# CogSP/CoEvoNet

Hardware: NVIDIA B200
Metric: mpe_env_steps_per_sec (higher is better)
Workload: dtype f32

## Files before the change

coevonet_b200/csrc/rollout_lockstep.cu:

```cuda
#include <stdlib.h>

#include <cuda_fp16.h>

#include "rollout_common.cuh"
#include "tc_common.cuh"

namespace cev {

constexpr int LS_ST_FIELDS = 16;
constexpr int LS_OBS_PAD = 12;
constexpr int LS_L1S = 132;

struct LsBuffers {
    double* st;
    double* acc;
    float* min_gap;
    int32_t* goal;
    float* obs;
    int32_t* act;
    float* gap;
    __half* w2split;
    uint32_t* wmax;
    float* oscale;
    double* l1stats;
    float2* l1ms;
    double* ml1stats;
};

static size_t ls_align(size_t x) { return (x + 255) & ~(size_t)255; }

static size_t ls_carve(void* base, int64_t N, int K, int P, LsBuffers* b) {
    size_t off = 0;
    char* p = static_cast<char*>(base);
    auto take = [&](size_t bytes) {
        void* r = p ? p + off : nullptr;
        off += ls_align(bytes);
        return r;
    };
    LsBuffers t;
    t.w2split = static_cast<__half*>(take((size_t)2 * K * 2 * H2 * H1 * sizeof(__half)));
    t.wmax = static_cast<uint32_t*>(take((size_t)2 * K * sizeof(uint32_t)));
    t.oscale = static_cast<float*>(take((size_t)2 * K * 2 * sizeof(float)));
    t.st = static_cast<double*>(take((size_t)LS_ST_FIELDS * N * sizeof(double)));
    t.acc = static_cast<double*>(take((size_t)3 * N * sizeof(double)));
    t.min_gap = static_cast<float*>(take((size_t)N * sizeof(float)));
    t.goal = static_cast<int32_t*>(take((size_t)N * sizeof(int32_t)));
    t.obs = static_cast<float*>(take((size_t)3 * N * LS_OBS_PAD * sizeof(float)));
    t.act = static_cast<int32_t*>(take((size_t)3 * N * sizeof(int32_t)));
    t.gap = static_cast<float*>(take((size_t)3 * N * sizeof(float)));
    t.l1stats = static_cast<double*>(take((size_t)2 * K * LS_L1S * sizeof(double)));
    t.l1ms = static_cast<float2*>(take((size_t)2 * N * sizeof(float2)));
    t.ml1stats = static_cast<double*>(take((size_t)P * LS_L1S * sizeof(double)));
    if (b) *b = t;
    return off;
}

__device__ __forceinline__ void ls_store_state(const LsBuffers& b, int64_t N, int64_t ep, const EnvState& s) {
// ... 137 lines not shown
    p.b.acc[p.N + ep] = rg;
    p.b.acc[2 * p.N + ep] = sum_adv;
    p.b.min_gap[ep] = min_gap;
    ls_store_state(p.b, p.N, ep, s);
    if (!ls_store_obs(p.b, p.N, ep, s, p.K, p.E, p.opp_seat) && p.status) atomicOr(p.status, CEV_STATUS_NONFINITE);
}

struct LsPrepParams {
    const float* opp[2];
    int64_t opp_pitch[2];
    int seat[2];
    int K;
    __half* w2split;
    uint32_t* wmax;
    float* oscale;
    double* l1stats;
};

__device__ __forceinline__ int ls_scale_exp(float bound, int target) {
    if (!(bound > 0.f) || !isfinite(bound)) return 0;
    const int s = target - ilogbf(bound);
    return s < -40 ? -40 : (s > 40 ? 40 : s);
}

__global__ void __launch_bounds__(256) ls_wmax_kernel(const LsPrepParams p) {
    const int oi = blockIdx.y / p.K, k = blockIdx.y % p.K;
    const FcOffsets o = fc_offsets(seat_in_dim(p.seat[oi]));
    const float4* src = reinterpret_cast<const float4*>(p.opp[oi] + (int64_t)k * p.opp_pitch[oi] + o.fc2w);
    float m = 0.f;
    for (int f = blockIdx.x * blockDim.x + threadIdx.x; f < H2 * H1 / 4; f += gridDim.x * blockDim.x) {
// ... 62 lines not shown
        }
#pragma unroll
        for (int o = 16; o > 0; o >>= 1) s += __shfl_xor_sync(0xffffffffu, s, o);
        if (lane == 0) {
            out[11 + a * 11 + b] = s / H1;
            out[11 + b * 11 + a] = s / H1;
        }
    }
}

__global__ void __launch_bounds__(512) ls_l1stats_kernel(const LsPrepParams p) {
    const int oi = blockIdx.x / p.K, k = blockIdx.x % p.K;
    const int in = seat_in_dim(p.seat[oi]);
    const float* row = p.opp[oi] + (int64_t)k * p.opp_pitch[oi];
    ls_l1stats_row(row, in, p.l1stats + (size_t)blockIdx.x * LS_L1S);
    __shared__ float red[2][16];
    const int t = threadIdx.x;
    float g = fabsf(row[H1 * in + H1 + t]), be = fabsf(row[H1 * in + 2 * H1 + t]);
#pragma unroll
    for (int off = 16; off > 0; off >>= 1) {
        g = fmaxf(g, __shfl_xor_sync(0xffffffffu, g, off));
        be = fmaxf(be, __shfl_xor_sync(0xffffffffu, be, off));
    }
    if ((t & 31) == 0) {
        red[0][t >> 5] = g;
        red[1][t >> 5] = be;
    }
    __syncthreads();
    if (t == 0) {
        for (int w = 1; w < 16; ++w) {
            g = fmaxf(g, red[0][w]);
            be = fmaxf(be, red[1][w]);
        }
        const int sx = ls_scale_exp(22.63f * g + be, 13);
        const int sw = ls_scale_exp(__uint_as_float(p.wmax[blockIdx.x]), 14);
        p.oscale[blockIdx.x * 2 + 0] = ldexpf(1.0f, sx);
        p.oscale[blockIdx.x * 2 + 1] = ldexpf(1.0f, -(sx + sw));
    }
}

__global__ void __launch_bounds__(512) ls_member_l1stats_kernel(const float* __restrict__ members, int64_t pitch, int in,
                                                                double* __restrict__ out) {
    ls_l1stats_row(members + (int64_t)blockIdx.x * pitch, in, out + (size_t)blockIdx.x * LS_L1S);
}

#ifndef LS_GRID_OPP_DEFAULT
#define LS_GRID_OPP_DEFAULT 0
#endif
#ifndef LS_GRID_MEM_DEFAULT
#define LS_GRID_MEM_DEFAULT 0
#endif
constexpr int LS_BT = 16;
constexpr int LS_TAIL_FLOATS = 2056;
constexpr int LS_W1A_FLOATS = H1 * IN_GOOD + 3 * H1;

constexpr int OP_THREADS = 448;
constexpr int OP_PROD = 256;
constexpr int OP_BM = 128, OP_BN = 256, OP_BK = 64, OP_KT = H1 / OP_BK;
constexpr uint32_t OP_A_BYTES = OP_BM * OP_BK * 2;
constexpr uint32_t OP_B_BYTES = OP_BN * OP_BK * 2;
constexpr uint32_t OP_STAGE_BYTES = 2 * OP_A_BYTES + 2 * OP_B_BYTES;
constexpr int OP_STAGES = 2;
constexpr size_t OP_OFF_W1A = (size_t)OP_STAGES * OP_STAGE_BYTES;
constexpr size_t OP_OFF_TAIL = OP_OFF_W1A + (size_t)LS_W1A_FLOATS * 4;
constexpr size_t OP_OFF_BAR = OP_OFF_TAIL + (size_t)LS_TAIL_FLOATS * 4;
constexpr size_t OP_SMEM_MAX = 232448;
constexpr size_t OP_SLACK = OP_SMEM_MAX - (OP_OFF_BAR + 128);
constexpr size_t OP_SMEM = OP_SMEM_MAX;
constexpr uint32_t OP_IDESC = (1u << 4) | ((uint32_t)(OP_BN >> 3) << 17) | ((uint32_t)(OP_BM >> 4) << 24);

struct LsOppParams {
    const float* opp[2];
    int64_t opp_pitch[2];
    int seat[2];
    int K, E, n_tiles, n_jobs;
    int64_t PE;
    int64_t N;
    const float* obs;
    int32_t* act;
    float* gap;
    const float2* l1ms;
    const float* oscale;
    int32_t* status;
    float* logits;
};

template <int IN>
__device__ __forceinline__ void op_produce_chunk(const float* __restrict__ w1a, const float (&x)[4][IN_GOOD],
                                                 const float (&mean)[4], const float (&rstd)[4], float sx, int kt, int c,
                                                 int lane, unsigned char* __restrict__ a_hi,
                                                 unsigned char* __restrict__ a_lo) {
    const float* fc1b = w1a + H1 * IN;
    const float* ln1g = fc1b + H1;
    const float* ln1b = ln1g + H1;
    const int k0 = kt * OP_BK + c * 8;
    uint32_t hi[4][4], lo[4][4];
#pragma unroll
    for (int half = 0; half < 2; ++half) {
        const float4 bb = *reinterpret_cast<const float4*>(fc1b + k0 + 4 * half);
        const float4 gg = *reinterpret_cast<const float4*>(ln1g + k0 + 4 * half);
        const float4 ee = *reinterpret_cast<const float4*>(ln1b + k0 + 4 * half);
        const float bq[4] = {bb.x, bb.y, bb.z, bb.w}, gq[4] = {gg.x * sx, gg.y * sx, gg.z * sx, gg.w * sx},
                    eq[4] = {ee.x * sx, ee.y * sx, ee.z * sx, ee.w * sx};
        float hv[4][4];
#pragma unroll
        for (int qq = 0; qq < 4; ++qq) {
            float w[IN];
            const float2* wr = reinterpret_cast<const float2*>(w1a + (k0 + 4 * half + qq) * IN);
#pragma unroll
            for (int i2 = 0; i2 < IN / 2; ++i2) {
                const float2 v = wr[i2];
                w[2 * i2] = v.x;
                w[2 * i2 + 1] = v.y;
            }
#pragma unroll
            for (int j = 0; j < 4; ++j) {
                float pre = 0.f;
#pragma unroll
                for (int i = 0; i < IN; ++i) pre = fmaf(w[i], x[j][i], pre);
                pre += bq[qq];
                hv[j][qq] = fmaxf(fmaf((pre - mean[j]) * rstd[j], gq[qq], eq[qq]), 0.f);
            }
        }
#pragma unroll
        for (int j = 0; j < 4; ++j)
#pragma unroll
            for (int pr = 0; pr < 2; ++pr) {
                const __half2 h2 = __floats2half2_rn(hv[j][2 * pr], hv[j][2 * pr + 1]);
                const float2 hf = __half22float2(h2);
                const __half2 l2 = __floats2half2_rn(hv[j][2 * pr] - hf.x, hv[j][2 * pr + 1] - hf.y);
                hi[j][2 * half + pr] = *reinterpret_cast<const uint32_t*>(&h2);
                lo[j][2 * half + pr] = *reinterpret_cast<const uint32_t*>(&l2);
            }
    }
#pragma unroll
    for (int j = 0; j < 4; ++j) {
        const int r = lane + 32 * j;
        const int off = r * 128 + ((c ^ (r & 7)) << 4);
        *reinterpret_cast<uint4*>(a_hi + off) = make_uint4(hi[j][0], hi[j][1], hi[j][2], hi[j][3]);
        *reinterpret_cast<uint4*>(a_lo + off) = make_uint4(lo[j][0], lo[j][1], lo[j][2], lo[j][3]);
    }
}

struct Geo {
    static constexpr uint32_t B_BYTES = OP_B_BYTES;
    static constexpr uint32_t STAGE_BYTES = OP_STAGE_BYTES;
    static constexpr int STAGES = OP_STAGES;
    static constexpr int ROWS_PER_JOB = OP_BM;
    static constexpr uint32_t N_FULL = OP_PROD / 32 + 1;
    static constexpr uint32_t N_TEMPTY = 4;
};

__global__ void __launch_bounds__(OP_THREADS, 1)
ls_opp_kernel(const __grid_constant__ CUtensorMap map_b, const LsOppParams p) {
    const int job0 = (int)blockIdx.x;
    const int job_stride = (int)gridDim.x;
    extern __shared__ unsigned char op_raw[];
    const uint32_t pad = (1024u - (smem_u32(op_raw) & 1023u)) & 1023u;
    if (pad > OP_SLACK) __trap();
    unsigned char* base = op_raw + pad;
    unsigned char* stage_mem = base;
    float* w1a = reinterpret_cast<float*>(base + OP_OFF_W1A);
    float* tail = reinterpret_cast<float*>(base + OP_OFF_TAIL);
    uint64_t* bar_full = reinterpret_cast<uint64_t*>(base + OP_OFF_BAR);
    uint64_t* bar_empty = bar_full + Geo::STAGES;
    uint64_t* bar_tfull = bar_empty + Geo::STAGES;
    uint64_t* bar_tempty = bar_tfull + 2;
    uint32_t* tmem_slot = reinterpret_cast<uint32_t*>(bar_tempty + 2);
    int* flag = reinterpret_cast<int*>(tmem_slot + 1);

    const int warp = threadIdx.x >> 5, lane = threadIdx.x & 31;

    if (threadIdx.x == 0) {
        *flag = 0;
        for (int i = 0; i < Geo::STAGES; ++i) {
            tc_mbar_init(bar_full + i, Geo::N_FULL);
            tc_mbar_init(bar_empty + i, 1);
        }
        for (int i = 0; i < 2; ++i) {
            tc_mbar_init(bar_tfull + i, 1);
            tc_mbar_init(bar_tempty + i, Geo::N_TEMPTY);
        }
        asm volatile("fence.mbarrier_init.release.cluster;\n" ::: "memory");
    }
    if (warp == 13) {
        asm volatile("tcgen05.alloc.cta_group::1.sync.aligned.shared::cta.b32 [%0], %1;\n" ::"r"(
                         tc_smem_u32(tmem_slot)),
                     "r"(512u)
                     : "memory");
        asm volatile("tcgen05.relinquish_alloc_permit.cta_group::1.sync.aligned;\n" ::: "memory");
    }
    asm volatile("tcgen05.fence::before_thread_sync;\n" ::: "memory");
    __syncthreads();
    asm volatile("tcgen05.fence::after_thread_sync;\n" ::: "memory");
    const uint32_t tmem_base = *tmem_slot;
    const int jobs_per_ok = p.n_tiles;

    if (warp < 4) {
        const int q = warp;
        uint32_t pass = 0;
        int cur_ok = -1;
        const float* b2 = tail;
        const float* g2 = tail + H2;
        const float* be2 = tail + 2 * H2;
        const float* w3 = tail + 3 * H2;
        const float* b3 = tail + 3 * H2 + NACT * H2;
        for (int job = job0; job < p.n_jobs; job += job_stride, ++pass) {
            const int okey = job / jobs_per_ok, tile = job % jobs_per_ok;
            const int oi = okey / p.K, k = okey % p.K;
            const int seat = oi ? p.seat[1] : p.seat[0];
            if (okey != cur_ok) {
                const float* row = (oi ? p.opp[1] : p.opp[0]) + (int64_t)k * (oi ? p.opp_pitch[1] : p.opp_pitch[0]);
                const float4* src = reinterpret_cast<const float4*>(row + fc_offsets(seat_in_dim(seat)).fc2b);
                asm volatile("bar.sync 2, 128;\n" ::: "memory");
                for (int f = threadIdx.x; f < LS_TAIL_FLOATS / 4; f += 128)
                    reinterpret_cast<float4*>(tail)[f] = __ldg(src + f);
                asm volatile("bar.sync 2, 128;\n" ::: "memory");
                cur_ok = okey;
            }
            const float unscale = __ldg(p.oscale + okey * 2 + 1);
            const int64_t j = (int64_t)tile * Geo::ROWS_PER_JOB + q * 32 + lane;
            const bool valid = j < p.PE;
            const int64_t jj = valid ? j : p.PE - 1;
            const int64_t ep = ((jj / p.E) * p.K + k) * p.E + (jj % p.E);
            const uint32_t as = pass & 1, ause = pass >> 1;
            tc_mbar_wait(bar_tfull + as, ause & 1);
            asm volatile("tcgen05.fence::after_thread_sync;\n" ::: "memory");
            const uint32_t taddr = tmem_base + ((uint32_t)(q * 32) << 16) + as * OP_BN;
            float sum = 0.f;
#pragma unroll 1
            for (int c0 = 0; c0 < OP_BN; c0 += 32) {
                uint32_t v[32];
                tmem_ld32(taddr + c0, v);
#pragma unroll
                for (int i = 0; i < 32; i += 4) {
                    const float4 bb = *reinterpret_cast<const float4*>(b2 + c0 + i);
                    sum += fmaf(__uint_as_float(v[i]), unscale, bb.x);
                    sum += fmaf(__uint_as_float(v[i + 1]), unscale, bb.y);
                    sum += fmaf(__uint_as_float(v[i + 2]), unscale, bb.z);
                    sum += fmaf(__uint_as_float(v[i + 3]), unscale, bb.w);
                }
            }
            const float mean = sum * (1.0f / H2);
// ... 34 lines not shown
                        const float x = fmaf(__uint_as_float(v[i + u]), unscale, bq[u]) - mean;
                        h[u] = fmaxf(fmaf(x * rstd, gq[u], eq[u]), 0.f);
                    }
#pragma unroll
                    for (int a = 0; a < NACT; ++a) {
                        const float4 ww = *reinterpret_cast<const float4*>(w3 + a * H2 + c);
                        lg[a] = fmaf(ww.x, h[0], lg[a]);
                        lg[a] = fmaf(ww.y, h[1], lg[a]);
                        lg[a] = fmaf(ww.z, h[2], lg[a]);
                        lg[a] = fmaf(ww.w, h[3], lg[a]);
                    }
                }
            }
            asm volatile("tcgen05.fence::before_thread_sync;\n" ::: "memory");
            __syncwarp();
            if (lane == 0) tc_mbar_arrive(bar_tempty + as);
            bool fin = isfinite(mean) && isfinite(var);
#pragma unroll
            for (int a = 0; a < NACT; ++a) {
                lg[a] += b3[a];
                fin = fin && isfinite(lg[a]);
            }
            float gap;
            const int a = argmax_first5(lg, gap);
            if (valid) {
                if (!fin) *flag = 1;
                p.act[(int64_t)seat * p.N + ep] = a;
                p.gap[(int64_t)seat * p.N + ep] = gap;
                if (p.logits) {
#pragma unroll
                    for (int u = 0; u < NACT; ++u) p.logits[((int64_t)seat * p.N + ep) * NACT + u] = lg[u];
                }
            }
        }
    } else if (warp < 12) {
        const int pt = threadIdx.x - 128;
        const int c = pt >> 5;
        int cur_ok = -1;
        uint32_t it = 0;
        for (int job = job0; job < p.n_jobs; job += job_stride) {
            const int okey = job / jobs_per_ok, tile = job % jobs_per_ok;
            const int oi = okey / p.K, k = okey % p.K;
            const int seat = oi ? p.seat[1] : p.seat[0];
            const int in = seat_in_dim(seat);
            const float* row = (oi ? p.opp[1] : p.opp[0]) + (int64_t)k * (oi ? p.opp_pitch[1] : p.opp_pitch[0]);
            if (okey != cur_ok) {
                asm volatile("bar.sync 1, 256;\n" ::: "memory");
                const int n4 = (H1 * in + 3 * H1) / 4;
                for (int f = pt; f < n4; f += OP_PROD)
                    reinterpret_cast<float4*>(w1a)[f] = __ldg(reinterpret_cast<const float4*>(row) + f);
                asm volatile("bar.sync 1, 256;\n" ::: "memory");
                cur_ok = okey;
            }
            const float sx = __ldg(p.oscale + okey * 2);
            float x[4][IN_GOOD];
            int64_t epj[4];
#pragma unroll
            for (int j = 0; j < 4; ++j) {
                const int64_t jrow = (int64_t)tile * Geo::ROWS_PER_JOB + lane + 32 * j;
                const int64_t jj = jrow < p.PE ? jrow : p.PE - 1;
                const int64_t ep = ((jj / p.E) * p.K + k) * p.E + (jj % p.E);
                epj[j] = ep;
                const float4* src = reinterpret_cast<const float4*>(p.obs + ((int64_t)seat * p.N + ep) * LS_OBS_PAD);
                const float4 v0 = __ldg(src), v1 = __ldg(src + 1), v2 = __ldg(src + 2);
                x[j][0] = v0.x; x[j][1] = v0.y; x[j][2] = v0.z; x[j][3] = v0.w;
                x[j][4] = v1.x; x[j][5] = v1.y; x[j][6] = v1.z; x[j][7] = v1.w;
                x[j][8] = v2.x; x[j][9] = v2.y;
            }
            float mean[4], rstd[4];
#pragma unroll
            for (int j = 0; j < 4; ++j) {
                const float2 v = __ldg(p.l1ms + (int64_t)oi * p.N + epj[j]);
                mean[j] = v.x;
                rstd[j] = v.y;
            }
            for (int kt = 0; kt < OP_KT; ++kt, ++it) {
                const uint32_t st = it % Geo::STAGES, use = it / Geo::STAGES;
                if (use > 0) tc_mbar_wait(bar_empty + st, (use - 1) & 1);
                unsigned char* a_hi = stage_mem + (size_t)st * Geo::STAGE_BYTES;
                unsigned char* a_lo = a_hi + OP_A_BYTES;
#if !(defined(CEV_EXP) && (CEV_EXP & 1))
                if (in == IN_GOOD) {
                    op_produce_chunk<IN_GOOD>(w1a, x, mean, rstd, sx, kt, c, lane, a_hi, a_lo);
                } else {
                    op_produce_chunk<IN_ADV>(w1a, x, mean, rstd, sx, kt, c, lane, a_hi, a_lo);
                }
#endif
                asm volatile("fence.proxy.async.shared::cta;\n" ::: "memory");
                __syncwarp();
                if (lane == 0) tc_mbar_arrive(bar_full + st);
            }
        }
    } else if (warp == 12) {
        if (lane == 0) {
            uint32_t it = 0;
            for (int job = job0; job < p.n_jobs; job += job_stride) {
                const int okey = job / jobs_per_ok;
                for (int kt = 0; kt < OP_KT; ++kt, ++it) {
                    const uint32_t st = it % Geo::STAGES, use = it / Geo::STAGES;
                    if (use > 0) tc_mbar_wait(bar_empty + st, (use - 1) & 1);
                    unsigned char* b_hi = stage_mem + (size_t)st * Geo::STAGE_BYTES + 2 * OP_A_BYTES;
#if defined(CEV_EXP) && (CEV_EXP & 2)
                    tc_mbar_arrive(bar_full + st);
                    (void)b_hi;
#else
                    tc_mbar_expect_tx(bar_full + st, 2 * OP_B_BYTES);
                    tma_load_2d(b_hi, &map_b, bar_full + st, kt * OP_BK, (okey * 2 + 0) * H2);
                    tma_load_2d(b_hi + OP_B_BYTES, &map_b, bar_full + st, kt * OP_BK, (okey * 2 + 1) * H2);
#endif
                }
            }
        }
    } else {
        const uint32_t stage_base = tc_smem_u32(stage_mem);
        uint32_t it = 0, pass = 0;
        for (int job = job0; job < p.n_jobs; job += job_stride, ++pass) {
            const uint32_t as = pass & 1, ause = pass >> 1;
            if (ause > 0) tc_mbar_wait(bar_tempty + as, (ause - 1) & 1);
            asm volatile("tcgen05.fence::after_thread_sync;\n" ::: "memory");
            const uint32_t d_tmem = tmem_base + as * OP_BN;
            for (int kt = 0; kt < OP_KT; ++kt, ++it) {
                const uint32_t st = it % Geo::STAGES, use = it / Geo::STAGES;
                tc_mbar_wait(bar_full + st, use & 1);
                asm volatile("tcgen05.fence::after_thread_sync;\n" ::: "memory");
                {
                    const uint32_t s_addr = stage_base + st * Geo::STAGE_BYTES;
                    tc_issue_ktile_3xf16(d_tmem, umma_desc_sw128(s_addr), umma_desc_sw128(s_addr + OP_A_BYTES),
                                          umma_desc_sw128(s_addr + 2 * OP_A_BYTES),
                                          umma_desc_sw128(s_addr + 2 * OP_A_BYTES + Geo::B_BYTES), OP_IDESC, kt ? 1u : 0u,
                                          tc_smem_u32(bar_empty + st));
                    if (kt == OP_KT - 1) tc_commit_elected(tc_smem_u32(bar_tfull + as));
                }
                __syncwarp();
            }
        }
    }
    asm volatile("tcgen05.fence::before_thread_sync;\n" ::: "memory");
    __syncthreads();
    if (threadIdx.x == 0 && *flag && p.status) atomicOr(p.status, CEV_STATUS_NONFINITE);
    if (warp == 13)
        asm volatile("tcgen05.dealloc.cta_group::1.sync.aligned.b32 %0, %1;\n" ::"r"(tmem_base), "r"(512u) : "memory");
}

}

#include "ls_member_tc.cuh"

// ... 65 lines not shown
    ls_carve(ws, N, p.K, p.P, &b);
    const int ms = p.member_seat;
    c->ms = ms;
    const int seat_of[2] = {ms == 0 ? 1 : 0, ms == 2 ? 1 : 2};

    LsPrepParams pp{};
    for (int oi = 0; oi < 2; ++oi) {
        pp.opp[oi] = p.opp[oi];
        pp.opp_pitch[oi] = p.opp_pitch[oi];
        pp.seat[oi] = seat_of[oi];
    }
    pp.K = p.K;
    pp.w2split = b.w2split;
    pp.wmax = b.wmax;
    pp.oscale = b.oscale;
    pp.l1stats = b.l1stats;
    CEV_CUDA(cudaMemsetAsync(b.wmax, 0, (size_t)2 * p.K * sizeof(uint32_t), stream));
    ls_wmax_kernel<<<dim3(32, 2 * p.K), 256, 0, stream>>>(pp);
    ls_split_w2_kernel<<<dim3(32, 2 * p.K), 256, 0, stream>>>(pp);
    ls_l1stats_kernel<<<2 * p.K, 512, 0, stream>>>(pp);
    ls_member_l1stats_kernel<<<p.P, 512, 0, stream_m>>>(p.members, p.member_pitch, seat_in_dim(ms), b.ml1stats);

    const FcOffsets om = fc_offsets(seat_in_dim(ms));
    {
        cuuint64_t dims[3] = {(cuuint64_t)H1, (cuuint64_t)H2, (cuuint64_t)p.P};
        cuuint64_t strides[2] = {(cuuint64_t)H1 * 4, (cuuint64_t)p.member_pitch * 4};
        cuuint32_t box[3] = {MT_BK, H2, 1};
        cuuint32_t estr[3] = {1, 1, 1};
        CUresult r = encode(&c->map_wtc, CU_TENSOR_MAP_DATA_TYPE_FLOAT32, 3, const_cast<float*>(p.members + om.fc2w), dims,
                            strides, box, estr, CU_TENSOR_MAP_INTERLEAVE_NONE, CU_TENSOR_MAP_SWIZZLE_128B,
// ... 43 lines not shown
        op.opp[oi] = p.opp[oi];
        op.opp_pitch[oi] = p.opp_pitch[oi];
        op.seat[oi] = seat_of[oi];
    }
    op.K = p.K;
    op.E = p.E;
    op.PE = (int64_t)p.P * p.E;
    op.n_tiles = (int)((op.PE + OP_BM - 1) / OP_BM);
    op.n_jobs = 2 * p.K * op.n_tiles;
    op.N = N;
    op.obs = b.obs;
    op.act = b.act;
    op.gap = b.gap;
    op.l1ms = b.l1ms;
    op.oscale = b.oscale;
    op.status = p.status;

    LsMemberTcParams& tp = c->tp;
    tp = LsMemberTcParams{};
    tp.members = p.members;
    tp.pitch = p.member_pitch;
    tp.KE = KE;
    tp.n_chunks = n_chunks;
    tp.seat = ms;
    tp.n_jobs = (int)c->member_ctas;
    tp.N = N;
    tp.obs = b.obs + (int64_t)ms * N * LS_OBS_PAD;
    tp.act = b.act + (int64_t)ms * N;
    tp.gap = b.gap + (int64_t)ms * N;
    tp.l1stats = b.ml1stats;
// ... 185 lines not shown
```

coevonet_b200/csrc/tc_common.cuh:

```cuda
#pragma once

#include <cuda.h>

#include "common.cuh"

namespace cev {

__device__ __forceinline__ uint32_t tc_smem_u32(const void* p) { return (uint32_t)__cvta_generic_to_shared(p); }

__device__ __forceinline__ void tc_mbar_init(uint64_t* bar, uint32_t count) {
    asm volatile("mbarrier.init.shared::cta.b64 [%0], %1;\n" ::"r"(tc_smem_u32(bar)), "r"(count) : "memory");
}
__device__ __forceinline__ void tc_mbar_expect_tx(uint64_t* bar, uint32_t bytes) {
    asm volatile("mbarrier.arrive.expect_tx.shared::cta.b64 _, [%0], %1;\n" ::"r"(tc_smem_u32(bar)), "r"(bytes)
                 : "memory");
}
__device__ __forceinline__ void tc_mbar_arrive(uint64_t* bar) {
    asm volatile("mbarrier.arrive.shared::cta.b64 _, [%0];\n" ::"r"(tc_smem_u32(bar)) : "memory");
}
__device__ __forceinline__ bool tc_mbar_try(uint64_t* bar, uint32_t parity) {
    uint32_t ok;
    asm volatile(
        "{\n.reg .pred p;\nmbarrier.try_wait.parity.shared::cta.b64 p, [%1], %2;\nselp.u32 %0, 1, 0, p;\n}\n"
        : "=r"(ok)
// ... 135 lines not shown
        "@pe tcgen05.mma.cta_group::1.kind::f16 [%0], %1, %3, %7, pt;\n"
        "@pe tcgen05.mma.cta_group::1.kind::f16 [%0], al1, bh1, %7, pt;\n"
        "@pe tcgen05.mma.cta_group::1.kind::f16 [%0], ah1, bl1, %7, pt;\n"
        "@pe tcgen05.mma.cta_group::1.kind::f16 [%0], ah1, bh1, %7, pt;\n"
        "@pe tcgen05.mma.cta_group::1.kind::f16 [%0], al2, bh2, %7, pt;\n"
        "@pe tcgen05.mma.cta_group::1.kind::f16 [%0], ah2, bl2, %7, pt;\n"
        "@pe tcgen05.mma.cta_group::1.kind::f16 [%0], ah2, bh2, %7, pt;\n"
        "@pe tcgen05.mma.cta_group::1.kind::f16 [%0], al3, bh3, %7, pt;\n"
        "@pe tcgen05.mma.cta_group::1.kind::f16 [%0], ah3, bl3, %7, pt;\n"
        "@pe tcgen05.mma.cta_group::1.kind::f16 [%0], ah3, bh3, %7, pt;\n"
        "@pe tcgen05.commit.cta_group::1.mbarrier::arrive::one.shared::cluster.b64 [%6];\n"
        "}\n" ::"r"(d_tmem),
        "l"(a_hi), "l"(a_lo), "l"(b_hi), "l"(b_lo), "r"(accumulate), "r"(bar_empty), "r"(idesc)
        : "memory");
}
__device__ __forceinline__ void tc_commit_elected(uint32_t bar) {
    asm volatile(
        "{\n.reg .pred pe;\nelect.sync _|pe, 0xffffffff;\n"
        "@pe tcgen05.commit.cta_group::1.mbarrier::arrive::one.shared::cluster.b64 [%0];\n}\n" ::"r"(bar)
        : "memory");
}

typedef CUresult (*EncodeTiledFn)(CUtensorMap*, CUtensorMapDataType, cuuint32_t, void*, const cuuint64_t*,
                                  const cuuint64_t*, const cuuint32_t*, const cuuint32_t*, CUtensorMapInterleave,
                                  CUtensorMapSwizzle, CUtensorMapL2promotion, CUtensorMapFloatOOBfill);

static inline EncodeTiledFn get_encode_fn() {
    static EncodeTiledFn fn = nullptr;
    if (!fn) {
        void* ptr = nullptr;
// ... 10 lines not shown
```

Before: 127.1 million.

## Move opponent first-layer matmul onto tensor cores with TMEM-resident activations

Moves the opponent network's first layer off the CUDA cores and onto tcgen05 MMAs. A prep kernel pre-scales and splits fc1 weights (with the bias folded in) into swizzled fp16 hi/lo images. A new MMA warp computes layer-1 in 64-column chunks into tensor memory; producer warps apply LayerNorm and ReLU, then store fp16 activations back to TMEM with tcgen05.st. The layer-2 GEMM then reads its A operand from TMEM, which removes A-tile staging in shared memory and the per-row scalar FMA loop. In exchange it adds another warp and more barriers, and the fp16 split of layer-1 inputs may cost some precision.

```diff
diff --git a/coevonet_b200/csrc/rollout_lockstep.cu b/coevonet_b200/csrc/rollout_lockstep.cu
--- a/coevonet_b200/csrc/rollout_lockstep.cu
+++ b/coevonet_b200/csrc/rollout_lockstep.cu
@@ -10,6 +10,10 @@
 constexpr int LS_ST_FIELDS = 16;
 constexpr int LS_OBS_PAD = 12;
 constexpr int LS_L1S = 132;
+constexpr int LS_OSC = 4;
+constexpr int LS_W1_TILE = 128 * 128;
+constexpr int LS_W1IMG_BYTES = 2 * LS_W1_TILE + 2 * H1 * 4;
+constexpr int LS_W1_BIAS = 10;
 
 struct LsBuffers {
     double* st;
@@ -22,6 +26,7 @@
     __half* w2split;
     uint32_t* wmax;
     float* oscale;
+    unsigned char* w1img;
     double* l1stats;
     float2* l1ms;
     double* ml1stats;
@@ -40,7 +45,8 @@
     LsBuffers t;
     t.w2split = static_cast<__half*>(take((size_t)2 * K * 2 * H2 * H1 * sizeof(__half)));
     t.wmax = static_cast<uint32_t*>(take((size_t)2 * K * sizeof(uint32_t)));
-    t.oscale = static_cast<float*>(take((size_t)2 * K * 2 * sizeof(float)));
+    t.oscale = static_cast<float*>(take((size_t)2 * K * LS_OSC * sizeof(float)));
+    t.w1img = static_cast<unsigned char*>(take((size_t)2 * K * LS_W1IMG_BYTES));
     t.st = static_cast<double*>(take((size_t)LS_ST_FIELDS * N * sizeof(double)));
     t.acc = static_cast<double*>(take((size_t)3 * N * sizeof(double)));
     t.min_gap = static_cast<float*>(take((size_t)N * sizeof(float)));
@@ -208,6 +214,7 @@
     __half* w2split;
     uint32_t* wmax;
     float* oscale;
+    unsigned char* w1img;
     double* l1stats;
 };
 
@@ -300,29 +307,65 @@
     const int in = seat_in_dim(p.seat[oi]);
     const float* row = p.opp[oi] + (int64_t)k * p.opp_pitch[oi];
     ls_l1stats_row(row, in, p.l1stats + (size_t)blockIdx.x * LS_L1S);
-    __shared__ float red[2][16];
+    __shared__ float red[3][16];
+    __shared__ float scl[2];
     const int t = threadIdx.x;
-    float g = fabsf(row[H1 * in + H1 + t]), be = fabsf(row[H1 * in + 2 * H1 + t]);
+    float w[16];
+#pragma unroll
+    for (int i = 0; i < 16; ++i) w[i] = i < in ? row[t * in + i] : (i == LS_W1_BIAS ? row[H1 * in + t] : 0.f);
+    float g = fabsf(row[H1 * in + H1 + t]), be = fabsf(row[H1 * in + 2 * H1 + t]), wm = 0.f;
+#pragma unroll
+    for (int i = 0; i < 16; ++i) wm = fmaxf(wm, fabsf(w[i]));
 #pragma unroll
     for (int off = 16; off > 0; off >>= 1) {
         g = fmaxf(g, __shfl_xor_sync(0xffffffffu, g, off));
         be = fmaxf(be, __shfl_xor_sync(0xffffffffu, be, off));
+        wm = fmaxf(wm, __shfl_xor_sync(0xffffffffu, wm, off));
     }
     if ((t & 31) == 0) {
         red[0][t >> 5] = g;
         red[1][t >> 5] = be;
+        red[2][t >> 5] = wm;
     }
     __syncthreads();
     if (t == 0) {
         for (int w = 1; w < 16; ++w) {
             g = fmaxf(g, red[0][w]);
             be = fmaxf(be, red[1][w]);
+            wm = fmaxf(wm, red[2][w]);
         }
         const int sx = ls_scale_exp(22.63f * g + be, 13);
         const int sw = ls_scale_exp(__uint_as_float(p.wmax[blockIdx.x]), 14);
-        p.oscale[blockIdx.x * 2 + 0] = ldexpf(1.0f, sx);
-        p.oscale[blockIdx.x * 2 + 1] = ldexpf(1.0f, -(sx + sw));
-    }
+        const int sw1 = ls_scale_exp(wm, 14);
+        p.oscale[blockIdx.x * LS_OSC + 0] = ldexpf(1.0f, sx);
+        p.oscale[blockIdx.x * LS_OSC + 1] = ldexpf(1.0f, -(sx + sw));
+        p.oscale[blockIdx.x * LS_OSC + 2] = ldexpf(1.0f, -sw1);
+        p.oscale[blockIdx.x * LS_OSC + 3] = 0.f;
+        scl[0] = ldexpf(1.0f, sx);
+        scl[1] = ldexpf(1.0f, sw1);
+    }
+    __syncthreads();
+    unsigned char* img = p.w1img + (size_t)blockIdx.x * LS_W1IMG_BYTES;
+    uint32_t hi[8], lo[8];
+#pragma unroll
+    for (int pr = 0; pr < 8; ++pr) {
+        const float v0 = w[2 * pr] * scl[1], v1 = w[2 * pr + 1] * scl[1];
+        const __half2 h2 = __floats2half2_rn(v0, v1);
+        const float2 hf = __half22float2(h2);
+        const __half2 l2 = __floats2half2_rn(v0 - hf.x, v1 - hf.y);
+        hi[pr] = *reinterpret_cast<const uint32_t*>(&h2);
+        lo[pr] = *reinterpret_cast<const uint32_t*>(&l2);
+    }
+    const int r = t & 127, c0 = 2 * (t >> 7);
+#pragma unroll
+    for (int c = 0; c < 2; ++c) {
+        const int off = r * 128 + (((c0 + c) ^ (r & 7)) << 4);
+        *reinterpret_cast<uint4*>(img + off) = make_uint4(hi[4 * c], hi[4 * c + 1], hi[4 * c + 2], hi[4 * c + 3]);
+        *reinterpret_cast<uint4*>(img + LS_W1_TILE + off) = make_uint4(lo[4 * c], lo[4 * c + 1], lo[4 * c + 2], lo[4 * c + 3]);
+    }
+    float* ge = reinterpret_cast<float*>(img + 2 * LS_W1_TILE);
+    ge[t] = row[H1 * in + H1 + t] * scl[0];
+    ge[H1 + t] = row[H1 * in + 2 * H1 + t] * scl[0];
 }
 
 __global__ void __launch_bounds__(512) ls_member_l1stats_kernel(const float* __restrict__ members, int64_t pitch, int in,
@@ -338,22 +381,27 @@
 #endif
 constexpr int LS_BT = 16;
 constexpr int LS_TAIL_FLOATS = 2056;
-constexpr int LS_W1A_FLOATS = H1 * IN_GOOD + 3 * H1;
-
-constexpr int OP_THREADS = 448;
+
+constexpr int OP_THREADS = 480;
 constexpr int OP_PROD = 256;
 constexpr int OP_BM = 128, OP_BN = 256, OP_BK = 64, OP_KT = H1 / OP_BK;
-constexpr uint32_t OP_A_BYTES = OP_BM * OP_BK * 2;
 constexpr uint32_t OP_B_BYTES = OP_BN * OP_BK * 2;
-constexpr uint32_t OP_STAGE_BYTES = 2 * OP_A_BYTES + 2 * OP_B_BYTES;
+constexpr uint32_t OP_STAGE_BYTES = 2 * OP_B_BYTES;
 constexpr int OP_STAGES = 2;
-constexpr size_t OP_OFF_W1A = (size_t)OP_STAGES * OP_STAGE_BYTES;
-constexpr size_t OP_OFF_TAIL = OP_OFF_W1A + (size_t)LS_W1A_FLOATS * 4;
+constexpr int OP_NB = 4;
+constexpr uint32_t OP_TM_L1 = OP_BN;
+constexpr size_t OP_OFF_W1 = (size_t)OP_STAGES * OP_STAGE_BYTES;
+constexpr size_t OP_OFF_A1 = OP_OFF_W1 + LS_W1IMG_BYTES;
+constexpr size_t OP_OFF_TAIL = OP_OFF_A1 + LS_W1_TILE;
 constexpr size_t OP_OFF_BAR = OP_OFF_TAIL + (size_t)LS_TAIL_FLOATS * 4;
 constexpr size_t OP_SMEM_MAX = 232448;
-constexpr size_t OP_SLACK = OP_SMEM_MAX - (OP_OFF_BAR + 128);
+constexpr size_t OP_SLACK = OP_SMEM_MAX - (OP_OFF_BAR + 256);
 constexpr size_t OP_SMEM = OP_SMEM_MAX;
+static_assert(OP_OFF_W1 % 1024 == 0 && OP_OFF_A1 % 1024 == 0, "swizzled tiles need 1 KB alignment");
+static_assert(OP_SLACK >= 1024, "opponent kernel exceeds the shared-memory limit");
+static_assert(OP_TM_L1 + OP_NB * OP_BK <= 512, "opponent kernel exceeds the tensor memory");
 constexpr uint32_t OP_IDESC = (1u << 4) | ((uint32_t)(OP_BN >> 3) << 17) | ((uint32_t)(OP_BM >> 4) << 24);
+constexpr uint32_t OP_IDESC1 = (1u << 4) | ((uint32_t)(OP_BK >> 3) << 17) | ((uint32_t)(OP_BM >> 4) << 24);
 
 struct LsOppParams {
     const float* opp[2];
@@ -367,106 +415,51 @@
     float* gap;
     const float2* l1ms;
     const float* oscale;
+    const unsigned char* w1img;
     int32_t* status;
     float* logits;
-};
-
-template <int IN>
-__device__ __forceinline__ void op_produce_chunk(const float* __restrict__ w1a, const float (&x)[4][IN_GOOD],
-                                                 const float (&mean)[4], const float (&rstd)[4], float sx, int kt, int c,
-                                                 int lane, unsigned char* __restrict__ a_hi,
-                                                 unsigned char* __restrict__ a_lo) {
-    const float* fc1b = w1a + H1 * IN;
-    const float* ln1g = fc1b + H1;
-    const float* ln1b = ln1g + H1;
-    const int k0 = kt * OP_BK + c * 8;
-    uint32_t hi[4][4], lo[4][4];
-#pragma unroll
-    for (int half = 0; half < 2; ++half) {
-        const float4 bb = *reinterpret_cast<const float4*>(fc1b + k0 + 4 * half);
-        const float4 gg = *reinterpret_cast<const float4*>(ln1g + k0 + 4 * half);
-        const float4 ee = *reinterpret_cast<const float4*>(ln1b + k0 + 4 * half);
-        const float bq[4] = {bb.x, bb.y, bb.z, bb.w}, gq[4] = {gg.x * sx, gg.y * sx, gg.z * sx, gg.w * sx},
-                    eq[4] = {ee.x * sx, ee.y * sx, ee.z * sx, ee.w * sx};
-        float hv[4][4];
-#pragma unroll
-        for (int qq = 0; qq < 4; ++qq) {
-            float w[IN];
-            const float2* wr = reinterpret_cast<const float2*>(w1a + (k0 + 4 * half + qq) * IN);
-#pragma unroll
-            for (int i2 = 0; i2 < IN / 2; ++i2) {
-                const float2 v = wr[i2];
-                w[2 * i2] = v.x;
-                w[2 * i2 + 1] = v.y;
-            }
-#pragma unroll
-            for (int j = 0; j < 4; ++j) {
-                float pre = 0.f;
-#pragma unroll
-                for (int i = 0; i < IN; ++i) pre = fmaf(w[i], x[j][i], pre);
-                pre += bq[qq];
-                hv[j][qq] = fmaxf(fmaf((pre - mean[j]) * rstd[j], gq[qq], eq[qq]), 0.f);
-            }
-        }
-#pragma unroll
-        for (int j = 0; j < 4; ++j)
-#pragma unroll
-            for (int pr = 0; pr < 2; ++pr) {
-                const __half2 h2 = __floats2half2_rn(hv[j][2 * pr], hv[j][2 * pr + 1]);
-                const float2 hf = __half22float2(h2);
-                const __half2 l2 = __floats2half2_rn(hv[j][2 * pr] - hf.x, hv[j][2 * pr + 1] - hf.y);
-                hi[j][2 * half + pr] = *reinterpret_cast<const uint32_t*>(&h2);
-                lo[j][2 * half + pr] = *reinterpret_cast<const uint32_t*>(&l2);
-            }
-    }
-#pragma unroll
-    for (int j = 0; j < 4; ++j) {
-        const int r = lane + 32 * j;
-        const int off = r * 128 + ((c ^ (r & 7)) << 4);
-        *reinterpret_cast<uint4*>(a_hi + off) = make_uint4(hi[j][0], hi[j][1], hi[j][2], hi[j][3]);
-        *reinterpret_cast<uint4*>(a_lo + off) = make_uint4(lo[j][0], lo[j][1], lo[j][2], lo[j][3]);
-    }
-}
-
-struct Geo {
-    static constexpr uint32_t B_BYTES = OP_B_BYTES;
-    static constexpr uint32_t STAGE_BYTES = OP_STAGE_BYTES;
-    static constexpr int STAGES = OP_STAGES;
-    static constexpr int ROWS_PER_JOB = OP_BM;
-    static constexpr uint32_t N_FULL = OP_PROD / 32 + 1;
-    static constexpr uint32_t N_TEMPTY = 4;
 };
 
 __global__ void __launch_bounds__(OP_THREADS, 1)
 ls_opp_kernel(const __grid_constant__ CUtensorMap map_b, const LsOppParams p) {
     const int job0 = (int)blockIdx.x;
     const int job_stride = (int)gridDim.x;
+    const int n_local = (p.n_jobs - job0 + job_stride - 1) / job_stride;
     extern __shared__ unsigned char op_raw[];
     const uint32_t pad = (1024u - (smem_u32(op_raw) & 1023u)) & 1023u;
     if (pad > OP_SLACK) __trap();
     unsigned char* base = op_raw + pad;
     unsigned char* stage_mem = base;
-    float* w1a = reinterpret_cast<float*>(base + OP_OFF_W1A);
+    unsigned char* w1img = base + OP_OFF_W1;
+    unsigned char* a1 = base + OP_OFF_A1;
     float* tail = reinterpret_cast<float*>(base + OP_OFF_TAIL);
     uint64_t* bar_full = reinterpret_cast<uint64_t*>(base + OP_OFF_BAR);
-    uint64_t* bar_empty = bar_full + Geo::STAGES;
-    uint64_t* bar_tfull = bar_empty + Geo::STAGES;
-    uint64_t* bar_tempty = bar_tfull + 2;
-    uint32_t* tmem_slot = reinterpret_cast<uint32_t*>(bar_tempty + 2);
+    uint64_t* bar_empty = bar_full + OP_STAGES;
+    uint64_t* bar_l1full = bar_empty + OP_STAGES;
+    uint64_t* bar_a2full = bar_l1full + OP_NB;
+    uint64_t* bar_bufempty = bar_a2full + OP_NB;
+    uint64_t* bar_a1full = bar_bufempty + OP_NB;
+    uint64_t* bar_tfull = bar_a1full + 2;
+    uint64_t* bar_tempty = bar_tfull + 1;
+    uint32_t* tmem_slot = reinterpret_cast<uint32_t*>(bar_tempty + 1);
     int* flag = reinterpret_cast<int*>(tmem_slot + 1);
 
     const int warp = threadIdx.x >> 5, lane = threadIdx.x & 31;
 
     if (threadIdx.x == 0) {
         *flag = 0;
-        for (int i = 0; i < Geo::STAGES; ++i) {
-            tc_mbar_init(bar_full + i, Geo::N_FULL);
+        for (int i = 0; i < OP_STAGES; ++i) {
+            tc_mbar_init(bar_full + i, 1);
             tc_mbar_init(bar_empty + i, 1);
         }
-        for (int i = 0; i < 2; ++i) {
-            tc_mbar_init(bar_tfull + i, 1);
-            tc_mbar_init(bar_tempty + i, Geo::N_TEMPTY);
-        }
+        for (int i = 0; i < OP_NB; ++i) {
+            tc_mbar_init(bar_l1full + i, 1);
+            tc_mbar_init(bar_a2full + i, OP_PROD / 32);
+            tc_mbar_init(bar_bufempty + i, 1);
+        }
+        for (int i = 0; i < 2; ++i) tc_mbar_init(bar_a1full + i, OP_PROD / 32);
+        tc_mbar_init(bar_tfull, 1);
+        tc_mbar_init(bar_tempty, 4);
         asm volatile("fence.mbarrier_init.release.cluster;\n" ::: "memory");
     }
     if (warp == 13) {
@@ -484,14 +477,13 @@
 
     if (warp < 4) {
         const int q = warp;
-        uint32_t pass = 0;
         int cur_ok = -1;
         const float* b2 = tail;
         const float* g2 = tail + H2;
         const float* be2 = tail + 2 * H2;
         const float* w3 = tail + 3 * H2;
         const float* b3 = tail + 3 * H2 + NACT * H2;
-        for (int job = job0; job < p.n_jobs; job += job_stride, ++pass) {
+        for (int jl = 0, job = job0; jl < n_local; ++jl, job += job_stride) {
             const int okey = job / jobs_per_ok, tile = job % jobs_per_ok;
             const int oi = okey / p.K, k = okey % p.K;
             const int seat = oi ? p.seat[1] : p.seat[0];
@@ -504,15 +496,14 @@
                 asm volatile("bar.sync 2, 128;\n" ::: "memory");
                 cur_ok = okey;
             }
-            const float unscale = __ldg(p.oscale + okey * 2 + 1);
-            const int64_t j = (int64_t)tile * Geo::ROWS_PER_JOB + q * 32 + lane;
+            const float unscale = __ldg(p.oscale + okey * LS_OSC + 1);
+            const int64_t j = (int64_t)tile * OP_BM + q * 32 + lane;
             const bool valid = j < p.PE;
             const int64_t jj = valid ? j : p.PE - 1;
             const int64_t ep = ((jj / p.E) * p.K + k) * p.E + (jj % p.E);
-            const uint32_t as = pass & 1, ause = pass >> 1;
-            tc_mbar_wait(bar_tfull + as, ause & 1);
+            tc_mbar_wait(bar_tfull, jl & 1);
             asm volatile("tcgen05.fence::after_thread_sync;\n" ::: "memory");
-            const uint32_t taddr = tmem_base + ((uint32_t)(q * 32) << 16) + as * OP_BN;
+            const uint32_t taddr = tmem_base + ((uint32_t)(q * 32) << 16);
             float sum = 0.f;
 #pragma unroll 1
             for (int c0 = 0; c0 < OP_BN; c0 += 32) {
@@ -577,7 +568,7 @@
             }
             asm volatile("tcgen05.fence::before_thread_sync;\n" ::: "memory");
             __syncwarp();
-            if (lane == 0) tc_mbar_arrive(bar_tempty + as);
+            if (lane == 0) tc_mbar_arrive(bar_tempty);
             bool fin = isfinite(mean) && isfinite(var);
 #pragma unroll
             for (int a = 0; a < NACT; ++a) {
@@ -598,60 +589,103 @@
         }
     } else if (warp < 12) {
         const int pt = threadIdx.x - 128;
-        const int c = pt >> 5;
-        int cur_ok = -1;
-        uint32_t it = 0;
-        for (int job = job0; job < p.n_jobs; job += job_stride) {
+        const int q = warp & 3, half = (warp - 4) >> 2;
+        const int r = q * 32 + lane;
+        const float* g1 = reinterpret_cast<const float*>(w1img + 2 * LS_W1_TILE);
+        const float* e1 = g1 + H1;
+        auto load_row = [&](int job, float (&x)[IN_GOOD], float2& ms) {
             const int okey = job / jobs_per_ok, tile = job % jobs_per_ok;
             const int oi = okey / p.K, k = okey % p.K;
             const int seat = oi ? p.seat[1] : p.seat[0];
-            const int in = seat_in_dim(seat);
-            const float* row = (oi ? p.opp[1] : p.opp[0]) + (int64_t)k * (oi ? p.opp_pitch[1] : p.opp_pitch[0]);
+            const int64_t jrow = (int64_t)tile * OP_BM + r;
+            const int64_t jj = jrow < p.PE ? jrow : p.PE - 1;
+            const int64_t ep = ((jj / p.E) * p.K + k) * p.E + (jj % p.E);
+            const float4* src = reinterpret_cast<const float4*>(p.obs + ((int64_t)seat * p.N + ep) * LS_OBS_PAD);
+            const float4 v0 = __ldg(src), v1 = __ldg(src + 1), v2 = __ldg(src + 2);
+            x[0] = v0.x; x[1] = v0.y; x[2] = v0.z; x[3] = v0.w;
+            x[4] = v1.x; x[5] = v1.y; x[6] = v1.z; x[7] = v1.w;
+            x[8] = v2.x; x[9] = v2.y;
+            ms = __ldg(p.l1ms + (int64_t)oi * p.N + ep);
+        };
+        float x[IN_GOOD];
+        float2 ms;
+        load_row(job0, x, ms);
+        int cur_ok = -1;
+        uint32_t it = 0;
+        for (int jl = 0, job = job0; jl < n_local; ++jl, job += job_stride) {
+            const int okey = job / jobs_per_ok;
             if (okey != cur_ok) {
                 asm volatile("bar.sync 1, 256;\n" ::: "memory");
-                const int n4 = (H1 * in + 3 * H1) / 4;
-                for (int f = pt; f < n4; f += OP_PROD)
-                    reinterpret_cast<float4*>(w1a)[f] = __ldg(reinterpret_cast<const float4*>(row) + f);
+                const uint4* src = reinterpret_cast<const uint4*>(p.w1img + (size_t)okey * LS_W1IMG_BYTES);
+                for (int f = pt; f < LS_W1IMG_BYTES / 16; f += OP_PROD) reinterpret_cast<uint4*>(w1img)[f] = __ldg(src + f);
+                asm volatile("fence.proxy.async.shared::cta;\n" ::: "memory");
                 asm volatile("bar.sync 1, 256;\n" ::: "memory");
                 cur_ok = okey;
             }
-            const float sx = __ldg(p.oscale + okey * 2);
-            float x[4][IN_GOOD];
-            int64_t epj[4];
-#pragma unroll
-            for (int j = 0; j < 4; ++j) {
-                const int64_t jrow = (int64_t)tile * Geo::ROWS_PER_JOB + lane + 32 * j;
-                const int64_t jj = jrow < p.PE ? jrow : p.PE - 1;
-                const int64_t ep = ((jj / p.E) * p.K + k) * p.E + (jj % p.E);
-                epj[j] = ep;
-                const float4* src = reinterpret_cast<const float4*>(p.obs + ((int64_t)seat * p.N + ep) * LS_OBS_PAD);
-                const float4 v0 = __ldg(src), v1 = __ldg(src + 1), v2 = __ldg(src + 2);
-                x[j][0] = v0.x; x[j][1] = v0.y; x[j][2] = v0.z; x[j][3] = v0.w;
-                x[j][4] = v1.x; x[j][5] = v1.y; x[j][6] = v1.z; x[j][7] = v1.w;
-                x[j][8] = v2.x; x[j][9] = v2.y;
-            }
-            float mean[4], rstd[4];
-#pragma unroll
-            for (int j = 0; j < 4; ++j) {
-                const float2 v = __ldg(p.l1ms + (int64_t)oi * p.N + epj[j]);
-                mean[j] = v.x;
-                rstd[j] = v.y;
-            }
+            float mx = 1.f;
+#pragma unroll
+            for (int i = 0; i < IN_GOOD; ++i) mx = fmaxf(mx, fabsf(x[i]));
+            const int se = ls_scale_exp(mx, 14);
+            const float ur = ldexpf(__ldg(p.oscale + okey * LS_OSC + 2), -se);
+            const float mean = ms.x, rstd = ms.y;
+            if (half == 0) {
+                const float sc = ldexpf(1.0f, se);
+                float av[16];
+#pragma unroll
+                for (int i = 0; i < 16; ++i) av[i] = i < IN_GOOD ? x[i] * sc : (i == LS_W1_BIAS ? sc : 0.f);
+                uint32_t hv[8], lv[8];
+#pragma unroll
+                for (int pr = 0; pr < 8; ++pr) {
+                    const __half2 h2 = __floats2half2_rn(av[2 * pr], av[2 * pr + 1]);
+                    const float2 hf = __half22float2(h2);
+                    const __half2 l2 = __floats2half2_rn(av[2 * pr] - hf.x, av[2 * pr + 1] - hf.y);
+                    hv[pr] = *reinterpret_cast<const uint32_t*>(&h2);
+                    lv[pr] = *reinterpret_cast<const uint32_t*>(&l2);
+                }
+                const int c0 = 4 * (jl & 1);
+                unsigned char* rowp = a1 + r * 128;
+                *reinterpret_cast<uint4*>(rowp + (((c0 + 0) ^ (r & 7)) << 4)) = make_uint4(hv[0], hv[1], hv[2], hv[3]);
+                *reinterpret_cast<uint4*>(rowp + (((c0 + 1) ^ (r & 7)) << 4)) = make_uint4(hv[4], hv[5], hv[6], hv[7]);
+                *reinterpret_cast<uint4*>(rowp + (((c0 + 2) ^ (r & 7)) << 4)) = make_uint4(lv[0], lv[1], lv[2], lv[3]);
+                *reinterpret_cast<uint4*>(rowp + (((c0 + 3) ^ (r & 7)) << 4)) = make_uint4(lv[4], lv[5], lv[6], lv[7]);
+                asm volatile("fence.proxy.async.shared::cta;\n" ::: "memory");
+            }
+            __syncwarp();
+            if (lane == 0) tc_mbar_arrive(bar_a1full + (jl & 1));
+            if (jl + 1 < n_local) load_row(job + job_stride, x, ms);
             for (int kt = 0; kt < OP_KT; ++kt, ++it) {
-                const uint32_t st = it % Geo::STAGES, use = it / Geo::STAGES;
-                if (use > 0) tc_mbar_wait(bar_empty + st, (use - 1) & 1);
-                unsigned char* a_hi = stage_mem + (size_t)st * Geo::STAGE_BYTES;
-                unsigned char* a_lo = a_hi + OP_A_BYTES;
-#if !(defined(CEV_EXP) && (CEV_EXP & 1))
-                if (in == IN_GOOD) {
-                    op_produce_chunk<IN_GOOD>(w1a, x, mean, rstd, sx, kt, c, lane, a_hi, a_lo);
-                } else {
-                    op_produce_chunk<IN_ADV>(w1a, x, mean, rstd, sx, kt, c, lane, a_hi, a_lo);
+                const uint32_t b = it % OP_NB;
+                tc_mbar_wait(bar_l1full + b, (it / OP_NB) & 1);
+                asm volatile("tcgen05.fence::after_thread_sync;\n" ::: "memory");
+                const uint32_t ta = tmem_base + ((uint32_t)(q * 32) << 16) + OP_TM_L1 + b * OP_BK + 32 * half;
+                uint32_t v[32];
+                tmem_ld32(ta, v);
+                const int k0 = kt * OP_BK + 32 * half;
+                uint32_t o[32];
+#pragma unroll
+                for (int i = 0; i < 32; i += 4) {
+                    const float4 gg = *reinterpret_cast<const float4*>(g1 + k0 + i);
+                    const float4 ee = *reinterpret_cast<const float4*>(e1 + k0 + i);
+                    const float gq[4] = {gg.x, gg.y, gg.z, gg.w}, eq[4] = {ee.x, ee.y, ee.z, ee.w};
+                    float y[4];
+#pragma unroll
+                    for (int u = 0; u < 4; ++u)
+                        y[u] = fmaxf(fmaf(fmaf(__uint_as_float(v[i + u]), ur, -mean) * rstd, gq[u], eq[u]), 0.f);
+#pragma unroll
+                    for (int pr = 0; pr < 2; ++pr) {
+                        const __half2 h2 = __floats2half2_rn(y[2 * pr], y[2 * pr + 1]);
+                        const float2 hf = __half22float2(h2);
+                        const __half2 l2 = __floats2half2_rn(y[2 * pr] - hf.x, y[2 * pr + 1] - hf.y);
+                        const int col = 16 * (i >> 4) + ((i & 15) >> 1) + pr;
+                        o[col] = *reinterpret_cast<const uint32_t*>(&h2);
+                        o[col + 8] = *reinterpret_cast<const uint32_t*>(&l2);
+                    }
                 }
-#endif
-                asm volatile("fence.proxy.async.shared::cta;\n" ::: "memory");
+                tmem_st32(ta, o);
+                asm volatile("tcgen05.wait::st.sync.aligned;\n" ::: "memory");
+                asm volatile("tcgen05.fence::before_thread_sync;\n" ::: "memory");
                 __syncwarp();
-                if (lane == 0) tc_mbar_arrive(bar_full + st);
+                if (lane == 0) tc_mbar_arrive(bar_a2full + b);
             }
         }
     } else if (warp == 12) {
@@ -660,40 +694,52 @@
             for (int job = job0; job < p.n_jobs; job += job_stride) {
                 const int okey = job / jobs_per_ok;
                 for (int kt = 0; kt < OP_KT; ++kt, ++it) {
-                    const uint32_t st = it % Geo::STAGES, use = it / Geo::STAGES;
+                    const uint32_t st = it % OP_STAGES, use = it / OP_STAGES;
                     if (use > 0) tc_mbar_wait(bar_empty + st, (use - 1) & 1);
-                    unsigned char* b_hi = stage_mem + (size_t)st * Geo::STAGE_BYTES + 2 * OP_A_BYTES;
-#if defined(CEV_EXP) && (CEV_EXP & 2)
-                    tc_mbar_arrive(bar_full + st);
-                    (void)b_hi;
-#else
+                    unsigned char* b_hi = stage_mem + (size_t)st * OP_STAGE_BYTES;
                     tc_mbar_expect_tx(bar_full + st, 2 * OP_B_BYTES);
                     tma_load_2d(b_hi, &map_b, bar_full + st, kt * OP_BK, (okey * 2 + 0) * H2);
                     tma_load_2d(b_hi + OP_B_BYTES, &map_b, bar_full + st, kt * OP_BK, (okey * 2 + 1) * H2);
-#endif
                 }
             }
         }
+    } else if (warp == 13) {
+        const uint32_t stage_base = tc_smem_u32(stage_mem);
+        uint32_t it = 0;
+        for (int jl = 0; jl < n_local; ++jl) {
+            if (jl > 0) tc_mbar_wait(bar_tempty, (jl - 1) & 1);
+            asm volatile("tcgen05.fence::after_thread_sync;\n" ::: "memory");
+            for (int kt = 0; kt < OP_KT; ++kt, ++it) {
+                const uint32_t st = it % OP_STAGES, b = it % OP_NB;
+                tc_mbar_wait(bar_full + st, (it / OP_STAGES) & 1);
+                tc_mbar_wait(bar_a2full + b, (it / OP_NB) & 1);
+                asm volatile("tcgen05.fence::after_thread_sync;\n" ::: "memory");
+                const uint32_t s_addr = stage_base + st * OP_STAGE_BYTES;
+                tc_issue_ktile_3xf16_ts(tmem_base, tmem_base + OP_TM_L1 + b * OP_BK, umma_desc_sw128(s_addr),
+                                        umma_desc_sw128(s_addr + OP_B_BYTES), OP_IDESC, kt ? 1u : 0u,
+                                        tc_smem_u32(bar_empty + st));
+                tc_commit_elected(tc_smem_u32(bar_bufempty + b));
+                if (kt == OP_KT - 1) tc_commit_elected(tc_smem_u32(bar_tfull));
+                __syncwarp();
+            }
+        }
     } else {
-        const uint32_t stage_base = tc_smem_u32(stage_mem);
-        uint32_t it = 0, pass = 0;
-        for (int job = job0; job < p.n_jobs; job += job_stride, ++pass) {
-            const uint32_t as = pass & 1, ause = pass >> 1;
-            if (ause > 0) tc_mbar_wait(bar_tempty + as, (ause - 1) & 1);
+        const uint32_t w1_base = tc_smem_u32(w1img), a1_base = tc_smem_u32(a1);
+        uint32_t it = 0;
+        for (int jl = 0; jl < n_local; ++jl) {
+            tc_mbar_wait(bar_a1full + (jl & 1), (jl >> 1) & 1);
             asm volatile("tcgen05.fence::after_thread_sync;\n" ::: "memory");
-            const uint32_t d_tmem = tmem_base + as * OP_BN;
+            const uint64_t a_hi = umma_desc_sw128(a1_base) + 4 * (jl & 1), a_lo = a_hi + 2;
             for (int kt = 0; kt < OP_KT; ++kt, ++it) {
-                const uint32_t st = it % Geo::STAGES, use = it / Geo::STAGES;
-                tc_mbar_wait(bar_full + st, use & 1);
-                asm volatile("tcgen05.fence::after_thread_sync;\n" ::: "memory");
-                {
-                    const uint32_t s_addr = stage_base + st * Geo::STAGE_BYTES;
-                    tc_issue_ktile_3xf16(d_tmem, umma_desc_sw128(s_addr), umma_desc_sw128(s_addr + OP_A_BYTES),
-                                          umma_desc_sw128(s_addr + 2 * OP_A_BYTES),
-                                          umma_desc_sw128(s_addr + 2 * OP_A_BYTES + Geo::B_BYTES), OP_IDESC, kt ? 1u : 0u,
-                                          tc_smem_u32(bar_empty + st));
-                    if (kt == OP_KT - 1) tc_commit_elected(tc_smem_u32(bar_tfull + as));
+                const uint32_t b = it % OP_NB, use = it / OP_NB;
+                if (use > 0) {
+                    tc_mbar_wait(bar_bufempty + b, (use - 1) & 1);
+                    asm volatile("tcgen05.fence::after_thread_sync;\n" ::: "memory");
                 }
+                const uint32_t w_addr = w1_base + (uint32_t)(kt & 1) * 64 * 128;
+                tc_issue_k16_3xf16(tmem_base + OP_TM_L1 + b * OP_BK, a_hi, a_lo, umma_desc_sw128(w_addr) + 2 * (kt >> 1),
+                                   umma_desc_sw128(w_addr + LS_W1_TILE) + 2 * (kt >> 1), OP_IDESC1,
+                                   tc_smem_u32(bar_l1full + b));
                 __syncwarp();
             }
         }
@@ -789,6 +835,7 @@
     pp.w2split = b.w2split;
     pp.wmax = b.wmax;
     pp.oscale = b.oscale;
+    pp.w1img = b.w1img;
     pp.l1stats = b.l1stats;
     CEV_CUDA(cudaMemsetAsync(b.wmax, 0, (size_t)2 * p.K * sizeof(uint32_t), stream));
     ls_wmax_kernel<<<dim3(32, 2 * p.K), 256, 0, stream>>>(pp);
@@ -862,6 +909,7 @@
     op.gap = b.gap;
     op.l1ms = b.l1ms;
     op.oscale = b.oscale;
+    op.w1img = b.w1img;
     op.status = p.status;
 
     LsMemberTcParams& tp = c->tp;
diff --git a/coevonet_b200/csrc/tc_common.cuh b/coevonet_b200/csrc/tc_common.cuh
--- a/coevonet_b200/csrc/tc_common.cuh
+++ b/coevonet_b200/csrc/tc_common.cuh
@@ -173,6 +173,64 @@
         "l"(a_hi), "l"(a_lo), "l"(b_hi), "l"(b_lo), "r"(accumulate), "r"(bar_empty), "r"(idesc)
         : "memory");
 }
+__device__ __forceinline__ void tc_issue_ktile_3xf16_ts(uint32_t d_tmem, uint32_t a_tmem, uint64_t b_hi, uint64_t b_lo,
+                                                         uint32_t idesc, uint32_t accumulate, uint32_t bar_empty) {
+    asm volatile(
+        "{\n"
+        ".reg .pred pe, pa, pt;\n"
+        ".reg .b32 ah0, ah1, ah2, ah3, al0, al1, al2, al3;\n"
+        ".reg .b64 bh1, bh2, bh3, bl1, bl2, bl3;\n"
+        "elect.sync _|pe, 0xffffffff;\n"
+        "setp.ne.b32 pa, %4, 0;\n"
+        "setp.eq.b32 pt, 0, 0;\n"
+        "add.u32 ah0, %1, 0;\n add.u32 ah1, %1, 16;\n add.u32 ah2, %1, 32;\n add.u32 ah3, %1, 48;\n"
+        "add.u32 al0, %1, 8;\n add.u32 al1, %1, 24;\n add.u32 al2, %1, 40;\n add.u32 al3, %1, 56;\n"
+        "add.s64 bh1, %2, 2;\n add.s64 bh2, %2, 4;\n add.s64 bh3, %2, 6;\n"
+        "add.s64 bl1, %3, 2;\n add.s64 bl2, %3, 4;\n add.s64 bl3, %3, 6;\n"
+        "@pe tcgen05.mma.cta_group::1.kind::f16 [%0], [al0], %2, %6, pa;\n"
+        "@pe tcgen05.mma.cta_group::1.kind::f16 [%0], [ah0], %3, %6, pt;\n"
+        "@pe tcgen05.mma.cta_group::1.kind::f16 [%0], [ah0], %2, %6, pt;\n"
+        "@pe tcgen05.mma.cta_group::1.kind::f16 [%0], [al1], bh1, %6, pt;\n"
+        "@pe tcgen05.mma.cta_group::1.kind::f16 [%0], [ah1], bl1, %6, pt;\n"
+        "@pe tcgen05.mma.cta_group::1.kind::f16 [%0], [ah1], bh1, %6, pt;\n"
+        "@pe tcgen05.mma.cta_group::1.kind::f16 [%0], [al2], bh2, %6, pt;\n"
+        "@pe tcgen05.mma.cta_group::1.kind::f16 [%0], [ah2], bl2, %6, pt;\n"
+        "@pe tcgen05.mma.cta_group::1.kind::f16 [%0], [ah2], bh2, %6, pt;\n"
+        "@pe tcgen05.mma.cta_group::1.kind::f16 [%0], [al3], bh3, %6, pt;\n"
+        "@pe tcgen05.mma.cta_group::1.kind::f16 [%0], [ah3], bl3, %6, pt;\n"
+        "@pe tcgen05.mma.cta_group::1.kind::f16 [%0], [ah3], bh3, %6, pt;\n"
+        "@pe tcgen05.commit.cta_group::1.mbarrier::arrive::one.shared::cluster.b64 [%5];\n"
+        "}\n" ::"r"(d_tmem),
+        "r"(a_tmem), "l"(b_hi), "l"(b_lo), "r"(accumulate), "r"(bar_empty), "r"(idesc)
+        : "memory");
+}
+__device__ __forceinline__ void tc_issue_k16_3xf16(uint32_t d_tmem, uint64_t a_hi, uint64_t a_lo, uint64_t b_hi, uint64_t b_lo,
+                                                   uint32_t idesc, uint32_t bar_full) {
+    asm volatile(
+        "{\n"
+        ".reg .pred pe, pf, pt;\n"
+        "elect.sync _|pe, 0xffffffff;\n"
+        "setp.ne.b32 pf, 0, 0;\n"
+        "setp.eq.b32 pt, 0, 0;\n"
+        "@pe tcgen05.mma.cta_group::1.kind::f16 [%0], %2, %3, %5, pf;\n"
+        "@pe tcgen05.mma.cta_group::1.kind::f16 [%0], %1, %4, %5, pt;\n"
+        "@pe tcgen05.mma.cta_group::1.kind::f16 [%0], %1, %3, %5, pt;\n"
+        "@pe tcgen05.commit.cta_group::1.mbarrier::arrive::one.shared::cluster.b64 [%6];\n"
+        "}\n" ::"r"(d_tmem),
+        "l"(a_hi), "l"(a_lo), "l"(b_hi), "l"(b_lo), "r"(idesc), "r"(bar_full)
+        : "memory");
+}
+__device__ __forceinline__ void tmem_st32(uint32_t taddr, const uint32_t (&v)[32]) {
+    asm volatile(
+        "tcgen05.st.sync.aligned.32x32b.x32.b32 [%0], "
+        "{%1, %2, %3, %4, %5, %6, %7, %8, %9, %10, %11, %12, %13, %14, %15, %16, "
+        "%17, %18, %19, %20, %21, %22, %23, %24, %25, %26, %27, %28, %29, %30, %31, %32};\n" ::"r"(taddr),
+        "r"(v[0]), "r"(v[1]), "r"(v[2]), "r"(v[3]), "r"(v[4]), "r"(v[5]), "r"(v[6]), "r"(v[7]), "r"(v[8]), "r"(v[9]),
+        "r"(v[10]), "r"(v[11]), "r"(v[12]), "r"(v[13]), "r"(v[14]), "r"(v[15]), "r"(v[16]), "r"(v[17]), "r"(v[18]),
+        "r"(v[19]), "r"(v[20]), "r"(v[21]), "r"(v[22]), "r"(v[23]), "r"(v[24]), "r"(v[25]), "r"(v[26]), "r"(v[27]),
+        "r"(v[28]), "r"(v[29]), "r"(v[30]), "r"(v[31])
+        : "memory");
+}
 __device__ __forceinline__ void tc_commit_elected(uint32_t bar) {
     asm volatile(
         "{\n.reg .pred pe;\nelect.sync _|pe, 0xffffffff;\n"
```

Result: no change. 128.3 million (median of 6 runs) (+0.9%).
